# littlespray/StreamFlow

Measured on AMD Instinct MI355X. Metric: flow_fields_per_sec, higher is better.
Workload: dtype f16x2 / f16 mixed (activations fp16; weights fp16 in 24 of the 45 contraction / depthwise layers, hi+lo in the rest; fp32 accumulate); fp16 correlation volumes; 1 GPU; sintel_440x1024_T4_iters15; clips_per_launch=8, device_pinning=single device, flow_fields_per_clip=3, parallelism=replicas1, hip_graph=True, preset=config2_mixed, corr_volume=fp16 cells, single f16 MFMA product, fp32 accumulate, gma=flash (fused recompute, 1 MFMA product(s) per logit)

## Files before the change

### include/streamflow_hip.h

```cpp
#ifndef STREAMFLOW_HIP_H
#define STREAMFLOW_HIP_H

#include <stddef.h>
#include <stdint.h>

#ifdef __cplusplus
extern "C" {
#endif

#define SF_VERSION 122

enum {
    SF_OK = 0,
    SF_ERR_BAD_ARG = -1,
    SF_ERR_UNSUPPORTED = -2,
    SF_ERR_HIP = -3
};

int sf_version(void);
const char* sf_last_error(void);

int sf_coords_grid(float* out, int batch, int ht, int wd, void* stream);

int sf_bilinear_sampler(const float* img, const float* coords, float* out, float* mask_out,
                        int M, int C, int Hi, int Wi, int Ho, int Wo, void* stream);
// ... 119 lines not shown
                            int64_t out_img_stride, void* out_koct, int64_t out_koct_img_stride, int n_img, int P, void* stream);

typedef struct SfFfnPair {
    const void* X; int64_t strideX; int64_t ldx;
    const void* wstream; int64_t wstream_bytes;
    const float* bias1; const float* bias2; const float* dw_w; const float* dw_b;
    float* C; int64_t strideC; int64_t ldc;
    void* C16; int64_t strideC16; int64_t ldc16;
    int32_t N, batch, K1, H, M2, pm1, pm2, mode, gelu_out, c16_partial;
    float alpha1, alpha2;
    int32_t x_group; int64_t x_group_stride;
    const float* R32; int64_t strideR32, ldr32, r32_group_stride;
} SfFfnPair;
int sf_ffn_pair(const SfFfnPair* p, void* stream);
int sf_ffn_pair_frags(int K1, int M2, int pm1, int pm2);

typedef struct SfSkTail {
    const void* X; int64_t strideX; int64_t ldx;
    const void* wstream; int64_t wstream_bytes;
    const float* bias1; const float* bias2; const float* bias3;
    float* Y; int64_t strideY; int64_t ldy;
    void* Y16; int64_t strideY16; int64_t ldy16;
    int32_t N, batch, C, H, M2, pm, gelu_out, y16_partial;
    float alpha1, alpha2, alpha3;
} SfSkTail;
int sf_sk_tail(const SfSkTail* p, void* stream);
int sf_sk_tail_frags(int C, int H, int M2, int pm);
int sf_sk_tail_layout(int C, int H, int M2, int pm, int* stage, int* group, int* pw_one_unit);

typedef struct SfTemporalBlock {
// ... 82 lines not shown
```

### streamflow_amd/_lib.py

```python
from __future__ import annotations

import ctypes as C
import os
from typing import Optional

import torch

_HERE = os.path.dirname(os.path.abspath(__file__))
LIB_PATH = os.environ.get("SF_HIP_LIB") or os.path.join(_HERE, "libstreamflow_hip.so")

LAYOUT_K_MAJOR, LAYOUT_K_MINOR, LAYOUT_SPLIT_F16, LAYOUT_F16_K_MINOR, LAYOUT_F16_K_MAJOR, LAYOUT_F16_KOCT, LAYOUT_SPLIT_KOCT = 0, 1, 2, 3, 4, 5, 6
PRECISION_FP32, PRECISION_F16X3, PRECISION_F16X2, PRECISION_F16 = 0, 1, 2, 3
EPI_NONE, EPI_GELU, EPI_RELU, EPI_RES, EPI_RES_GELU, EPI_RES_GELU_DW1, EPI_AXPY = range(7)
ALGO_AUTO, ALGO_TILED, ALGO_BSTAT = 0, 1, 2

_vp, _i, _i64, _f = C.c_void_p, C.c_int, C.c_int64, C.c_float


class SfGemm(C.Structure):
    _fields_ = [
        ("A", _vp), ("B", _vp), ("C", _vp), ("bias", _vp), ("R", _vp), ("dw_w", _vp), ("dw_b", _vp), ("gamma", _vp),
        ("M", C.c_int32), ("N", C.c_int32), ("K", C.c_int32), ("batch", C.c_int32),
        ("lda", _i64), ("ldb", _i64), ("ldc", _i64), ("ldr", _i64),
        ("strideA", _i64), ("strideB", _i64), ("strideC", _i64), ("strideR", _i64),
# ... 97 lines not shown
    "sf_corr_build_blocked32_ws_bytes": (_i64, [_i, _i, _i, _i]),
    "sf_corr_build_blocked32": (_i, [_vp, _vp, _i64, _i64, _vp, _i64, _i, _i, _i, _i, _i, _vp, _i64, _vp]),
    "sf_corr_lookup_blocked32": (_i, [_vp, _i64, _vp, _vp, _i64, _i, _i, _i, _i, _vp]),
    "sf_gemm": (_i, [C.POINTER(SfGemm), _vp]),
    "sf_gemm_split_ws_floats": (_i64, [_i, _i, _i, _i]),
    "sf_gma_flash_ws_bytes": (_i64, [_i, _i]),
    "sf_gma_flash_pack_qk": (_i, [_vp, _i64, _vp, _i64, _i, _i, _f, _i, _vp]),
    "sf_gma_flash_aggregate": (_i, [_vp, _i64, _vp, _i64, _vp, _i64, _vp, _vp, _i64, _vp, _i64, _i, _i, _i, _i, _vp]),
    "sf_gma_flash_aggregate_f16v": (_i, [_vp, _i64, _vp, _i64, _vp, _i64, _vp, _vp, _i64, _vp, _i64, _i, _i, _i, _i, _vp]),
    "sf_gma_flash_project_v": (_i, [_vp, _i64, _vp, _i64, _i64, _vp, _vp, _i, _f, _i, _i, _i, _vp]),
    "sf_gma_stored_p_bytes": (_i64, [_i, _i]),
    "sf_gma_flash_store_p": (_i, [_vp, _i64, _vp, _i64, _i, _i, _i, _vp]),
    "sf_gma_stored_aggregate": (_i, [_vp, _i64, _vp, _i64, _vp, _i, _i64, _vp, _i64, _vp, _vp, _i64, _vp, _i64, _i, _i, _vp]),
    "sf_ffn_pair": (_i, [C.POINTER(SfFfnPair), _vp]),
    "sf_ffn_pair_frags": (_i, [_i, _i, _i, _i]),
    "sf_sk_tail": (_i, [C.POINTER(SfSkTail), _vp]),
    "sf_sk_tail_frags": (_i, [_i, _i, _i, _i]),
    "sf_sk_tail_layout": (_i, [_i, _i, _i, _i, C.POINTER(C.c_int), C.POINTER(C.c_int), C.POINTER(C.c_int)]),
    "sf_temporal_block": (_i, [C.POINTER(SfTemporalBlock), _vp]),
    "sf_temporal_block_frags": (_i, [_i]),
    "sf_mask_upsample": (_i, [C.POINTER(SfMaskUpsample), _vp]),
    "sf_mask_upsample_frags": (_i, [_i]),
    "sf_softmax_rows": (_i, [_vp, _i64, _i, _vp, _vp]),
    "sf_splitk_combine": (_i, [_vp, _i64, _i, _i64, _vp, _i64, _vp, _vp, _i64, _i, _i64, _vp]),
    "sf_dwconv_res_gelu": (_i, [_vp, _i64, _vp, _vp, _vp, _i64, _i, _i, _i, _i, _i, _i, _i, _vp]),
    "sf_dwconv_res_gelu_f16in": (_i, [_vp, _i64, _vp, _vp, _vp, _i64, _i, _i, _i, _i, _i, _i, _vp]),
    "sf_layernorm_cm": (_i, [_vp, _i64, _vp, _vp, _vp, _i64, _vp, _i64, _i, _i, _i, _f, _vp]),
    "sf_temporal_attn": (_i, [_vp, _vp, _vp, _i, _i, _i, _i, _vp]),
    "sf_temporal_attn_f16in": (_i, [_vp, _vp, _vp, _i, _i, _i, _i, _vp]),
    "sf_pack_koct": (_i, [_vp, _i64, _i, _i, _i, _vp, _i64, _vp]),
# ... 69 lines not shown
```

### streamflow_amd/build.py

```python
from __future__ import annotations

import os
import shutil
import subprocess
import sys
from concurrent.futures import ThreadPoolExecutor

HERE = os.path.dirname(os.path.abspath(__file__))
CSRC = os.path.join(HERE, "csrc")
OBJ = os.path.join(CSRC, "build")
LIB = os.path.join(HERE, "libstreamflow_hip.so")
ASAN_OBJ = os.path.join(CSRC, "build_asan")
ASAN_LIB = os.path.join(HERE, "libstreamflow_hip_asan.so")
SOURCES = ["misc.hip", "corr.hip", "corr_blocked.hip", "corr_blocked32.hip", "conv.hip", "gemm.hip", "gemm_split.hip", "gemm_bstat.hip", "ffn_pair.hip", "sk_tail.hip", "temporal.hip", "mask_upsample.hip", "attn.hip", "encoder.hip", "tile_blend.hip"]
HEADERS = [os.path.join(CSRC, "sf_common.h"), os.path.join(CSRC, "gemm_epilogue.h"), os.path.join(CSRC, "split_operand.h"),
           os.path.join(HERE, "..", "include", "streamflow_hip.h")]
FLAGS = ["--offload-arch=gfx950", "-O3", "-std=c++17", "-fPIC", "-fno-slp-vectorize", "-Wall",
         "-Wno-unused-function",
         "-Rpass-analysis=kernel-resource-usage"]
HOT_KERNELS = ("gemm_bstat", "ffn_pair_kernel", "sk_tail_kernel", "gma_flash_pipe_kernel", "gma_pv_kernel", "temporal_block_kernel", "mask_upsample_kernel", "gemm_bdirect_kernel", "gma_flash_kernel", "flash_project_v_kernel", "dwconv_mfma_kernel",
               "corr_lookup_blocked_kernel", "corr_build_blocked_kernel", "corr_lookup_blocked32_kernel", "corr_build_blocked32_kernel", "temporal_attn_kernel", "layernorm_cm_split_kernel",
               "flash_pack_v_kernel")


def hipcc() -> str:
    exe = shutil.which("hipcc") or "/opt/rocm/bin/hipcc"
    if not os.path.exists(exe):
        raise RuntimeError("hipcc not found; libstreamflow_hip.so cannot be built")
    return exe


def _stale(target: str, deps) -> bool:
    if not os.path.exists(target):
        return True
    t = os.path.getmtime(target)
# ... 169 lines not shown
```

### streamflow_amd/engine.py

```python
from __future__ import annotations

import contextlib
import os
from dataclasses import dataclass, fields, replace
from typing import Dict, List, Optional, Sequence, Tuple

import torch

from . import _lib, ops
from .ops import (EPI_AXPY, EPI_GELU, EPI_NONE, EPI_RELU, EPI_RES, EPI_RES_GELU, EPI_RES_GELU_DW1, LAYOUT_F16_K_MINOR,
                  LAYOUT_K_MAJOR, LAYOUT_K_MINOR, PackedLinear, Planes, Workspace)

HDIM = 128
COR_PLANES = 324


@dataclass(frozen=True)
class EngineOptions:
    parallel_branches: bool = True
    split_solo: int = 2
    split_uneven: bool = False
    auto_split_k: bool = True
    attn_chunk_rows: int = 0
    attn_k_splits: int = 3
    corr_blocked: bool = True
    corr_blocked32: bool = True
    shadows: bool = True
    shadow_fused: bool = True
    hidden_f16: bool = True
    hidden_koct: bool = True
    split_handover: bool = False
    pw_fold: bool = True
    koct_io: bool = True
    x2_f16: bool = True
    flash_stats: bool = True
    ffn_pairs: bool = True
    project_v: bool = True
    temporal_block: bool = True
    sk_tail: bool = True
    sk_tail_all: bool = False
    head_pairs: bool = False
    mask_upsample: bool = True
    clock_probe_us: int = 0
    setup_overlap: bool = True
    gma_per_chain: bool = True
    hybrid_store_pct: int = 50
    stored_auto_px: int = 16384
    stored_auto_max_gb: int = 16
    stored_p_max_gb: int = 64
    max_plans: int = 4

# ... 16 lines not shown

class SKBlockWeights:

    def __init__(self, sd: Dict[str, torch.Tensor], prefix: str, device):
        g = lambda n: sd[prefix + "." + n]
        self.ffn1_0 = PackedLinear(g("ffn1.0.weight"), g("ffn1.0.bias"), device)
        self.ffn1_2 = PackedLinear(g("ffn1.2.weight"), g("ffn1.2.bias"), device)
        self.pw = PackedLinear(g("pw.weight"), g("pw.bias"), device)
        wpw = g("pw.weight")
        eye = torch.eye(wpw.shape[0], dtype=wpw.dtype, device=wpw.device).reshape(wpw.shape[0], wpw.shape[0], *wpw.shape[2:])
        self.pw_res = PackedLinear(wpw + eye, g("pw.bias"), device)
        self.ffn2_0 = PackedLinear(g("ffn2.0.weight"), g("ffn2.0.bias"), device)
        self.ffn2_2 = PackedLinear(g("ffn2.2.weight"), g("ffn2.2.bias"), device)
        self.pair1 = ops.PackedPair(self.ffn1_0, self.ffn1_2)
        self.pair2 = ops.PackedPair(self.ffn2_0, self.ffn2_2)
        self.tail = ops.PackedTail(self.pw_res, self.ffn2_0, self.ffn2_2)
        self.c_in, self.c_mid, self.c_out = self.ffn1_0.K, self.ffn1_0.M, self.ffn2_2.M
        f32 = lambda t: t.detach().to(device=device, dtype=torch.float32).contiguous()
        w0 = g("conv_list.0.weight")
        if w0.shape[-1] != 1:
            raise RuntimeError("SKBlock: first depthwise kernel must be 1x1 (k_conv=[1,K]), got %s" % (tuple(w0.shape),))
        self.dw1_w = f32(w0.reshape(-1))
        self.dw1_b = f32(g("conv_list.0.bias"))
        wk = g("conv_list.1.weight")
        self.k = int(wk.shape[-1])
        self.dwk_w = f32(wk.reshape(wk.shape[0], -1))
        self.dwk_b = f32(g("conv_list.1.bias"))
        self.dw_single = False


# ... 17 lines not shown
    assert 0 <= i0 and i0 + cnt <= X.n_img
    step = X.img_stride // (2 if X.f16 else 1)
    assert not X.f16 or X.img_stride % 2 == 0
    sh = _sub(X.shadow, i0, cnt) if X.shadow is not None else None
    return replace(X, off=X.off + i0 * step, n_img=cnt, shadow=sh)


def _part(buf: Planes, i0: int, cnt: int) -> Planes:
    return replace(buf, off=buf.off + i0 * buf.img_stride, n_img=cnt)


def hidden_f16_ok(cx: ops.Ctx, P: int) -> bool:
    return cx.precision in (ops.PRECISION_F16X2, ops.PRECISION_F16) and P % 4 == 0 and cx.hidden_f16


def run_skblock(W: SKBlockWeights, X: Planes, Y: Planes, hid: Planes, xa: Planes, xb: Planes, h: int, w: int,
                final_gelu: bool = False, cx: Optional[ops.Ctx] = None) -> None:
    cx = ops._cx(cx)
    C = W.c_in
    assert X.rows == C and Y.rows == W.c_out and X.n_img == Y.n_img
    a, b = _scratch(xa, X.n_img, C), _scratch(xb, X.n_img, C)
    fold = hidden_f16_ok(cx, X.P) and cx.pw_fold
    if fold and cx.x2_f16:
        a = _scratch(xa, X.n_img, C, f16=True)
    head_pairs = cx.head_pairs and X.group and X.shadow is not None and X.n_img * X.P >= 4 * 7040
    if cx.ffn_pairs and a.f16 and ((X.f16 and X.koct) or head_pairs) and ops.ffn_pair_ok(W.pair1, X, 1, cx):
        ops.ffn_pair(W.pair1, X, a, 1, dw_w=W.dw1_w, dw_b=W.dw1_b, cx=cx)
    else:
        hidden = _handover(cx, hid, X.n_img, W.c_mid, X.P, consumer_rows=C)
        ops.gemm(W.ffn1_0, X, hidden, EPI_GELU, cx=cx)
        ops.gemm(W.ffn1_2, hidden, a, EPI_RES_GELU_DW1, R=X, dw_w=W.dw1_w, dw_b=W.dw1_b, cx=cx)
    if fold:
        b16 = _scratch(xb, X.n_img, C, f16=True)
        ops.dwconv_res_gelu(a, W.dwk_w, W.dwk_b, b16, h, w, W.k, single=W.dw_single, cx=cx)
        if (ops.sk_tail_ok(W.tail, b16, Y, cx) and W.c_in <= 256 and X.n_img * X.P >= 4 * 7040) or \
                (cx.sk_tail_all and ops.sk_tail_ok(W.tail, b16, Y, cx)):
            ops.sk_tail(W.tail, b16, Y, gelu_out=final_gelu, cx=cx)
            return
        a4 = _handover(cx, xa, X.n_img, C, X.P, consumer_rows=W.c_mid)
        ops.gemm(W.pw_res, b16, a4, EPI_GELU, cx=cx)
    else:
        ops.dwconv_res_gelu(a, W.dwk_w, W.dwk_b, b, h, w, W.k, single=W.dw_single, cx=cx)
        a4 = _handover(cx, xa, X.n_img, C, X.P, consumer_rows=W.c_mid, allow_koct=False)
        ops.gemm(W.pw, b, a4, EPI_RES_GELU, R=b, cx=cx)
    pair2_pays = W.c_in <= 128 or W.pair2.products(cx) == (1, 1) or (W.c_out <= 16 and head_pairs)
    if X.n_img * X.P < 4 * 7040 and not X.group:
        pair2_pays = True
    if (cx.ffn_pairs and pair2_pays and a4.f16 and a4.koct and ops.ffn_pair_ok(W.pair2, a4, 0, cx) and (not Y.f16 or Y.koct)):
        ops.ffn_pair(W.pair2, a4, Y, 0, gelu_out=final_gelu, cx=cx)
        return
    hidden = _handover(cx, hid, X.n_img, W.c_mid, X.P, consumer_rows=W.c_out)
    ops.gemm(W.ffn2_0, a4, hidden, EPI_GELU, cx=cx)
    ops.gemm(W.ffn2_2, hidden, Y, EPI_GELU if final_gelu else EPI_NONE, cx=cx)


class HotPathWeights:

    def __init__(self, sd: Dict[str, torch.Tensor], device, T: Optional[int] = None):
        sd = {(k[7:] if k.startswith("module.") else k): v for k, v in sd.items()}
# ... 196 lines not shown
        if self.gma_mode not in ("auto", "matrix", "flash", "stored", "hybrid"):
            raise RuntimeError(f"gma_mode must be auto, matrix, flash, stored or hybrid, got {self.gma_mode!r}")
        self.flash_qk_products = (int(flash_qk_products or 0)
                                  or {ops.PRECISION_F16X2: 2, ops.PRECISION_F16: 1}.get(self.precision, 3))
        if self.flash_qk_products not in (1, 2, 3):
            raise RuntimeError(f"flash_qk_products must be 1, 2 or 3, got {self.flash_qk_products}")
        self._side = torch.cuda.Stream(device=self.device)
        if int(self.options.clock_probe_us) > 0:
            self._probe_stream = torch.cuda.Stream(device=self.device)
            self.clock_counts = torch.zeros(2, dtype=torch.int64, device=self.device)
        self._chain_streams = [torch.cuda.Stream(device=self.device) for _ in range(3)]
        self.split_solo = int(self.options.split_solo)
        self.W = HotPathWeights(state_dict, self.device, T)
        self.single_layers = tuple(single_layers or ())
        self.W.set_single("all" if self.single_layers == ("all",) else self.single_layers)
        if (self.options.ffn_pairs or self.options.sk_tail) and self.precision in (ops.PRECISION_F16X2, ops.PRECISION_F16):
            cxp = ops.Ctx(precision=self.precision)
            with torch.cuda.device(self.device):
                for b in HotPathWeights.SK_BLOCKS:
                    blk = getattr(self.W, b)
                    for pair in (blk.pair1, blk.pair2) if self.options.ffn_pairs else ():
                        if (pair.K1, pair.M2) in ops.PAIR_SHAPES[0] | ops.PAIR_SHAPES[1]:
                            pair.stream(*pair.products(cxp))
                    if self.options.sk_tail and blk.tail.built(blk.tail.products(cxp)):
                        blk.tail.stream(blk.tail.products(cxp))
                torch.cuda.synchronize(self.device)
        if self.options.mask_upsample and self.precision in (ops.PRECISION_F16X2, ops.PRECISION_F16) and self.W.mask_pack.built():
            with torch.cuda.device(self.device):
                self.W.mask_pack.stream(self.W.mask_pack.products(ops.Ctx(precision=self.precision)))
                torch.cuda.synchronize(self.device)
        if self.options.temporal_block and self.precision in (ops.PRECISION_F16X2, ops.PRECISION_F16) and self.W.temporal.built():
            pm = self.W.temporal.products(ops.Ctx(precision=self.precision))
            if pm is not None:
                with torch.cuda.device(self.device):
                    self.W.temporal.stream(pm)
                    torch.cuda.synchronize(self.device)
        self.use_graph = use_graph
        self._plans: Dict[Tuple[int, int, int, int], _Plan] = {}
# ... 21 lines not shown
                       corr_blocked=self.corr_blocked, corr_blocked32=self.corr_blocked32,
                       koct_io=self.options.koct_io and self.options.hidden_koct,
                       stored_p=((self.gma_mode in ("stored", "hybrid") or auto_stored) and self.options.flash_stats),
                       stored_frac=(1.0 if (self.gma_mode == "stored" or auto_stored) else float(self.options.hybrid_store_pct) / 100.0),
                       stored_p_max_bytes=int(self.options.stored_p_max_gb) << 30)
            pl.auto_stored = bool(auto_stored and pl.pbuf is not None)
        self._plans[key] = pl
        return pl

    def _ctx(self, pl: _Plan) -> ops.Ctx:
        o = self.options
        return ops.Ctx(precision=self.precision,
                       split_ws=pl.splitws.tensor().view(-1) if self.auto_split_k else None,
                       shadows=o.shadows, shadow_fused=o.shadow_fused, flash_stats=o.flash_stats,
                       hidden_f16=o.hidden_f16, hidden_koct=o.hidden_koct, split_handover=o.split_handover, pw_fold=o.pw_fold, x2_f16=o.x2_f16,
                       ffn_pairs=o.ffn_pairs, head_pairs=o.head_pairs, sk_tail=o.sk_tail, sk_tail_all=o.sk_tail_all)

    @staticmethod
    def _flash_ws_sub(pl: _Plan, i0: int, cnt: int) -> torch.Tensor:
        if i0 == 0 and cnt == pl.n:
            return pl.flash_ws
        ib = ops.gma_flash_img_bytes(pl.P)
        return pl.flash_ws[i0 * ib:(i0 + cnt) * ib]

    def _attention_rows(self, cx: ops.Ctx, pl: _Plan, i0: int, rows: int) -> None:
        P, n = pl.P, pl.n
        ops.gemm_raw(cx, A=pl.qk.ptr + 4 * i0, B=pl.qk.ptr + 4 * HDIM * P, C=pl.attn.data_ptr(), M=rows, N=P, K=HDIM,
                     batch=n, lda=P, ldb=P, ldc=P, strideA=pl.qk.img_stride, strideB=pl.qk.img_stride,
                     strideC=pl.attn_rows * P, a_layout=LAYOUT_K_MAJOR, b_layout=LAYOUT_K_MAJOR,
                     alpha=float(HDIM) ** -0.5, epilogue=EPI_NONE)
        if rows == pl.attn_rows:
# ... 303 lines not shown
```

### streamflow_amd/ops.py

```python
from __future__ import annotations

import ctypes as C
import math
import os
from dataclasses import dataclass, replace
from typing import Optional, Sequence

import torch

from . import _lib
from ._lib import (EPI_AXPY, EPI_GELU, EPI_NONE, EPI_RELU, EPI_RES, EPI_RES_GELU, EPI_RES_GELU_DW1,
                   LAYOUT_K_MAJOR, LAYOUT_K_MINOR, LAYOUT_SPLIT_F16, LAYOUT_F16_K_MINOR, PRECISION_F16, PRECISION_F16X2, PRECISION_F16X3,
                   PRECISION_FP32,
                   SfGemm)

PRECISION = PRECISION_F16X3
_PRECISION_NAMES = {"fp32": PRECISION_FP32, "f16x3": PRECISION_F16X3, "f16x2": PRECISION_F16X2, "f16": PRECISION_F16}


def set_precision(mode) -> int:
    global PRECISION
    prev = PRECISION
    PRECISION = _PRECISION_NAMES[mode] if isinstance(mode, str) else int(mode)
    if PRECISION not in (PRECISION_FP32, PRECISION_F16X3, PRECISION_F16X2, PRECISION_F16):
# ... 8 lines not shown

@dataclass(frozen=True)
class Ctx:
    precision: int
    split_ws: Optional[torch.Tensor] = None
    shadows: bool = True
    shadow_fused: bool = True
    flash_stats: bool = True
    hidden_f16: bool = True
    hidden_koct: bool = True
    split_handover: bool = False
    pw_fold: bool = True
    x2_f16: bool = True
    ffn_pairs: bool = True
    head_pairs: bool = False
    sk_tail: bool = True
    sk_tail_all: bool = False

    def no_split(self) -> "Ctx":
        return self if self.split_ws is None else replace(self, split_ws=None)


def _cx(cx: Optional["Ctx"]) -> "Ctx":
    return cx if cx is not None else Ctx(PRECISION)


class Profiler:

    def __init__(self):
        self.records = []
# ... 229 lines not shown
        h1, l1 = self._split(self.first, hp * 32, nk1 * 32)
        h2, l2 = self._split(self.second, nt2 * 16, hp * 32)
        dev = h1.device
        planes1 = [l1, h1] if pm1 == 2 else [h1]
        f1 = torch.stack([w.view(hp, 2, 16, nk1, 4, 8) for w in planes1], dim=0)
        f1 = f1.permute(1, 2, 4, 0, 5, 3, 6).reshape(hp, 2 * nk1 * pm1, 64 * 8)
        kq = torch.arange(4, device=dev).view(4, 1)
        i = torch.arange(8, device=dev).view(1, 8)
        perm = torch.where(i < 4, 4 * kq + i, 16 + 4 * kq + i - 4).reshape(-1)
        planes2 = [l2, h2] if pm2 == 2 else [h2]
        f2 = torch.stack([w.view(nt2, 16, hp, 32)[..., perm].reshape(nt2, 16, hp, 4, 8) for w in planes2], dim=0)
        f2 = f2.permute(3, 1, 0, 4, 2, 5).reshape(hp, nt2 * pm2, 64 * 8)
        pad = torch.zeros(hp, fpad - f1.shape[1] - f2.shape[1], 64 * 8, dtype=torch.float16, device=dev)
        st = torch.cat([f1, f2, pad], dim=1).contiguous().view(-1)
        assert st.numel() * 2 == hp * fpad * 1024
        self._streams[key] = st
        return st


class PackedTail:

    S = 16

    def __init__(self, pw_res: "PackedLinear", f0: "PackedLinear", f2: "PackedLinear"):
        assert pw_res.M == pw_res.K == f0.K and f0.M == f2.K and not (pw_res.conv3x3 or f0.conv3x3 or f2.conv3x3)
        self.layers = (pw_res, f0, f2)
        self.C, self.H, self.M2 = pw_res.K, f0.M, f2.M
        self._streams = {}

    def products(self, cx: "Ctx") -> Optional[int]:
# ... 293 lines not shown
        g.C16, g.strideC16, g.ldc16 = Y.ptr, Y.img_stride, Y.P
    else:
        g.C, g.strideC, g.ldc = Y.ptr, Y.img_stride, Y.P
        out_bytes = 4.0
        if Y.shadow is not None and cx.shadows:
            sh = Y.shadow
            g.C16, g.strideC16, g.ldc16 = sh.ptr, sh.img_stride, sh.P
            g.c16_partial = 1 if pair.M2 % 8 else 0
            out_bytes = 6.0
    n, P = X.n_img, X.P
    flops = 2.0 * n * P * (pair.K1 * pair.H + pair.H * pair.M2)
    mf = 2.0 * n * P * (pair.K1 * pair.H * pm1 + pair.H * pair.M2 * pm2)
    nbytes = n * P * (2.0 * pair.K1 * (2 if mode == 1 else 1) + out_bytes * pair.M2) + 2.0 * (pair.K1 * pair.H * pm1 + pair.H * pair.M2 * pm2)
    name = "ffn_pair" if not PROFILE_SHAPES else f"ffn_pair K{pair.K1} H{pair.H} M{pair.M2} b{n} m{mode}"
    _launch(name, flops, nbytes, lambda: _lib.check(_lib.load().sf_ffn_pair(C.byref(g), _lib.stream()), "sf_ffn_pair"),
            products=mf / flops)
    if g.C and not g.C16:
        refresh_shadow(Y, cx)


def new_shadow(X: Planes, device) -> Planes:
    assert not X.f16 and X.group == 0
    noct = (X.rows + 7) // 8
    base = torch.zeros(X.n_img * noct * X.P * 4, dtype=torch.float32, device=device)
    return Planes(base, 0, noct * X.P * 8, X.n_img, X.rows, X.P, f16=True, koct=True)


@on_tensor_device
def pack_koct(X: Planes, Y: Planes) -> None:
    assert Y.f16 and Y.koct and not X.f16 and X.group == 0 and (X.rows, X.P, X.n_img) == (Y.rows, Y.P, Y.n_img)
# ... 577 lines not shown
```

Baseline: 387.1 flow-fields/s.

## Add fused FFN chain kernel keeping hidden tile in registers across both GEMMs

Adds a new ffn_chain kernel that computes the two pointwise layers of an FFN block in one pass. Each hidden 32-row tile is produced by MFMA, passed through GELU, converted to f16 fragments and consumed straight away by the second GEMM. Weights stream through a three-stage LDS ring using buffer-load-to-LDS, and a mode-1 epilogue applies the residual, depthwise and GELU steps. This is meant to replace the existing ffn_pair path for suitable shapes and cut hidden-activation traffic, at the cost of high register pressure and more complex weight packing.

```diff
diff --git a/include/streamflow_hip.h b/include/streamflow_hip.h
--- a/include/streamflow_hip.h
+++ b/include/streamflow_hip.h
@@ -8,7 +8,7 @@
 extern "C" {
 #endif
 
-#define SF_VERSION 122
+#define SF_VERSION 123
 
 enum {
     SF_OK = 0,
@@ -158,6 +158,8 @@
 } SfFfnPair;
 int sf_ffn_pair(const SfFfnPair* p, void* stream);
 int sf_ffn_pair_frags(int K1, int M2, int pm1, int pm2);
+int sf_ffn_chain(const SfFfnPair* p, void* stream);
+int sf_ffn_chain_frags(int K1, int H, int M2, int pm1, int pm2);
 
 typedef struct SfSkTail {
     const void* X; int64_t strideX; int64_t ldx;
diff --git a/streamflow_amd/_lib.py b/streamflow_amd/_lib.py
--- a/streamflow_amd/_lib.py
+++ b/streamflow_amd/_lib.py
@@ -135,6 +135,8 @@
     "sf_gma_stored_aggregate": (_i, [_vp, _i64, _vp, _i64, _vp, _i, _i64, _vp, _i64, _vp, _vp, _i64, _vp, _i64, _i, _i, _vp]),
     "sf_ffn_pair": (_i, [C.POINTER(SfFfnPair), _vp]),
     "sf_ffn_pair_frags": (_i, [_i, _i, _i, _i]),
+    "sf_ffn_chain": (_i, [C.POINTER(SfFfnPair), _vp]),
+    "sf_ffn_chain_frags": (_i, [_i, _i, _i, _i, _i]),
     "sf_sk_tail": (_i, [C.POINTER(SfSkTail), _vp]),
     "sf_sk_tail_frags": (_i, [_i, _i, _i, _i]),
     "sf_sk_tail_layout": (_i, [_i, _i, _i, _i, C.POINTER(C.c_int), C.POINTER(C.c_int), C.POINTER(C.c_int)]),
diff --git a/streamflow_amd/build.py b/streamflow_amd/build.py
--- a/streamflow_amd/build.py
+++ b/streamflow_amd/build.py
@@ -12,13 +12,13 @@
 LIB = os.path.join(HERE, "libstreamflow_hip.so")
 ASAN_OBJ = os.path.join(CSRC, "build_asan")
 ASAN_LIB = os.path.join(HERE, "libstreamflow_hip_asan.so")
-SOURCES = ["misc.hip", "corr.hip", "corr_blocked.hip", "corr_blocked32.hip", "conv.hip", "gemm.hip", "gemm_split.hip", "gemm_bstat.hip", "ffn_pair.hip", "sk_tail.hip", "temporal.hip", "mask_upsample.hip", "attn.hip", "encoder.hip", "tile_blend.hip"]
+SOURCES = ["misc.hip", "corr.hip", "corr_blocked.hip", "corr_blocked32.hip", "conv.hip", "gemm.hip", "gemm_split.hip", "gemm_bstat.hip", "ffn_pair.hip", "ffn_chain.hip", "sk_tail.hip", "temporal.hip", "mask_upsample.hip", "attn.hip", "encoder.hip", "tile_blend.hip"]
 HEADERS = [os.path.join(CSRC, "sf_common.h"), os.path.join(CSRC, "gemm_epilogue.h"), os.path.join(CSRC, "split_operand.h"),
            os.path.join(HERE, "..", "include", "streamflow_hip.h")]
 FLAGS = ["--offload-arch=gfx950", "-O3", "-std=c++17", "-fPIC", "-fno-slp-vectorize", "-Wall",
          "-Wno-unused-function",
          "-Rpass-analysis=kernel-resource-usage"]
-HOT_KERNELS = ("gemm_bstat", "ffn_pair_kernel", "sk_tail_kernel", "gma_flash_pipe_kernel", "gma_pv_kernel", "temporal_block_kernel", "mask_upsample_kernel", "gemm_bdirect_kernel", "gma_flash_kernel", "flash_project_v_kernel", "dwconv_mfma_kernel",
+HOT_KERNELS = ("gemm_bstat", "ffn_pair_kernel", "ffn_chain_kernel", "sk_tail_kernel", "gma_flash_pipe_kernel", "gma_pv_kernel", "temporal_block_kernel", "mask_upsample_kernel", "gemm_bdirect_kernel", "gma_flash_kernel", "flash_project_v_kernel", "dwconv_mfma_kernel",
                "corr_lookup_blocked_kernel", "corr_build_blocked_kernel", "corr_lookup_blocked32_kernel", "corr_build_blocked32_kernel", "temporal_attn_kernel", "layernorm_cm_split_kernel",
                "flash_pack_v_kernel")
 
diff --git a/streamflow_amd/csrc/ffn_chain.hip b/streamflow_amd/csrc/ffn_chain.hip
--- /dev/null
+++ b/streamflow_amd/csrc/ffn_chain.hip
@@ -0,0 +1,383 @@
+#include "sf_common.h"
+#include <type_traits>
+
+namespace {
+
+typedef _Float16 f16x8 __attribute__((ext_vector_type(8)));
+typedef _Float16 f16x4 __attribute__((ext_vector_type(4)));
+typedef float f32x16 __attribute__((ext_vector_type(16)));
+typedef float f32x4 __attribute__((ext_vector_type(4)));
+typedef unsigned int u32x2 __attribute__((ext_vector_type(2)));
+typedef __attribute__((address_space(3))) void* lds_ptr;
+using sf::f32x2;
+
+constexpr int kThreads = 256, kWaves = 4;
+constexpr int BN = 128;
+constexpr int S = 16;
+constexpr int kStage = S * 1024;
+constexpr int RING = 3;
+constexpr int PCS = S / kWaves;
+constexpr int kOob = 1 << 30;
+constexpr int kMaxH = 960, kMaxM = 384;
+
+struct ChainArgs {
+    SfFfnPair p;
+    int ntile;
+    int nh;
+    int x_span;
+    int64_t w_bytes;
+};
+
+template <int N>
+__device__ __forceinline__ void wait_vm() { __builtin_amdgcn_s_waitcnt((N & 15) | 0x0F70 | ((N >> 4) << 14)); }
+
+template <int I, int N, class F>
+__device__ __forceinline__ void static_for(F&& f) {
+    if constexpr (I < N) {
+        f(std::integral_constant<int, I>{});
+        static_for<I + 1, N>(f);
+    }
+}
+
+template <int NP>
+__device__ __forceinline__ void gelu_poly_n(f32x2 (&x)[NP]) {
+    f32x2 xc[NP], t[NP], p[NP];
+#pragma unroll
+    for (int i = 0; i < NP; ++i) {
+        xc[i][0] = __builtin_amdgcn_fmed3f(x[i][0], -4.2426405f, 4.2426405f);
+        xc[i][1] = __builtin_amdgcn_fmed3f(x[i][1], -4.2426405f, 4.2426405f);
+        t[i] = xc[i] * xc[i];
+        p[i] = sf::splat2(1.12535e-10f);
+    }
+    constexpr float c[8] = {-1.074371e-08f, 4.5365834e-07f, -1.12924145e-05f, 0.0001871811f, -0.0022188f, 0.019636236f,
+                            -0.13269384f, 0.79780626f};
+#pragma unroll
+    for (int k = 0; k < 8; ++k)
+#pragma unroll
+        for (int i = 0; i < NP; ++i) p[i] = __builtin_elementwise_fma(p[i], t[i], sf::splat2(c[k]));
+#pragma unroll
+    for (int i = 0; i < NP; ++i) {
+        const f32x2 h = sf::splat2(0.5f) * __builtin_elementwise_max(x[i], sf::splat2(-4.2426405f));
+        x[i] = __builtin_elementwise_fma(h, xc[i] * p[i], h);
+    }
+}
+
+template <int NP>
+__device__ __forceinline__ void tile_to_frags(const f32x16& acc, float alpha, f16x8& f0, f16x8& f1) {
+#pragma unroll
+    for (int s = 0; s < 2; ++s) {
+        f16x8 h;
+#pragma unroll
+        for (int c = 0; c < 4; c += NP) {
+            f32x2 v[NP];
+#pragma unroll
+            for (int q = 0; q < NP; ++q) {
+                v[q][0] = alpha * acc[8 * s + 2 * (c + q)];
+                v[q][1] = alpha * acc[8 * s + 2 * (c + q) + 1];
+            }
+            gelu_poly_n<NP>(v);
+#pragma unroll
+            for (int q = 0; q < NP; ++q) {
+                h[2 * (c + q)] = (_Float16)v[q][0];
+                h[2 * (c + q) + 1] = (_Float16)v[q][1];
+            }
+        }
+        if (s == 0) f0 = h; else f1 = h;
+    }
+}
+
+constexpr int chain_regs(int NK1, int NM, int MODE) { return (MODE == 1 ? 2 * NM : NK1) * 4 + NM * 16; }
+
+template <int NK1, int NM, int PM1, int PM2, int MODE>
+__global__ __launch_bounds__(kThreads, chain_regs(NK1, NM, MODE) <= 212 ? 2 : 1) void ffn_chain_kernel(const ChainArgs a) {
+    const SfFfnPair& g = a.p;
+    constexpr int NX = MODE == 1 ? 2 * NM : NK1;
+    static_assert(NX >= NK1, "mode 1 needs M2 == K1");
+    constexpr int NA = NK1 * PM1, NB = 2 * NM * PM2, TF = NA + NB;
+    constexpr int U = (TF + S - 1) / S;
+    constexpr int GNP = chain_regs(NK1, NM, MODE) > 160 ? 2 : 4;
+    __shared__ __attribute__((aligned(1024))) char smem[RING * kStage + (kMaxH + kMaxM) * 4];
+    float* sb1 = reinterpret_cast<float*>(smem + RING * kStage);
+    float* sb2 = sb1 + kMaxH;
+    float* sdw = reinterpret_cast<float*>(smem);
+    float* sdb = sdw + kMaxM;
+    const int tid = threadIdx.x, lane = tid & 63;
+    const int wave = __builtin_amdgcn_readfirstlane(tid >> 6);
+    const int khalf = lane >> 5, l31 = lane & 31;
+    const int tile = blockIdx.x % a.ntile, z = blockIdx.x / a.ntile;
+    const int n = tile * BN + wave * 32 + l31, nc = min(n, g.N - 1);
+
+    const __amdgpu_buffer_rsrc_t rw = __builtin_amdgcn_make_buffer_rsrc(const_cast<void*>(g.wstream), 0, (int)a.w_bytes, 0x00020000);
+    const int last_stage = (int)(a.w_bytes / kStage) - 1;
+    auto issue_stage = [&](int s, int slot) {
+        const int sc = min(s, last_stage);
+#pragma unroll
+        for (int i = 0; i < PCS; ++i) {
+            const int piece = wave + kWaves * i;
+            __builtin_amdgcn_raw_ptr_buffer_load_lds(rw, (lds_ptr)(smem + slot * kStage + piece * 1024), 16, lane * 16,
+                                                     sc * kStage + piece * 1024, 0, 0);
+        }
+    };
+#pragma unroll
+    for (int i = 0; i < RING - 1; ++i) issue_stage(i, i);
+
+    for (int i = tid; i < a.nh * 32; i += kThreads) sb1[i] = (i < g.H && g.bias1) ? g.bias1[i] : 0.f;
+    for (int i = tid; i < NM * 32; i += kThreads) sb2[i] = (i < g.M2 && g.bias2) ? g.bias2[i] : 0.f;
+
+    const int noct = (g.K1 + 7) / 8;
+    const __amdgpu_buffer_rsrc_t rx = __builtin_amdgcn_make_buffer_rsrc(
+        const_cast<char*>(reinterpret_cast<const char*>(g.X)) + (int64_t)z * g.strideX * 2, 0, a.x_span, 0x00020000);
+    f16x8 x[NX];
+#pragma unroll
+    for (int s = 0; s < NX; ++s) {
+        const int oc = 2 * s + khalf;
+        x[s] = __builtin_bit_cast(f16x8, __builtin_amdgcn_raw_buffer_load_b128(rx, oc < noct ? (khalf * (int)g.ldx + nc) * 16 : kOob,
+                                                                              2 * s * (int)g.ldx * 16, 0));
+    }
+    wait_vm<0>();
+    __syncthreads();
+
+    int gs = 0, slot = 0;
+    auto run_unit = [&](auto&& body) {
+        static_for<0, U>([&](auto st_tag) {
+            constexpr int st = decltype(st_tag)::value;
+            issue_stage(gs + RING - 1, slot == 0 ? RING - 1 : slot - 1);
+            const char* sp = smem + slot * kStage + lane * 16;
+            static_for<0, S>([&](auto i_tag) {
+                constexpr int i = decltype(i_tag)::value;
+                body(std::integral_constant<int, st * S + i>{}, sp + i * 1024);
+            });
+            {
+                constexpr int nm = (TF - st * S) < 0 ? 0 : ((TF - st * S) > S ? S : (TF - st * S));
+                constexpr int kAhead = 3;
+                __builtin_amdgcn_sched_group_barrier(0x002, 2, 0);
+                __builtin_amdgcn_sched_group_barrier(0x100, nm < kAhead ? nm : kAhead, 0);
+#pragma unroll
+                for (int i = 0; i < nm; ++i) {
+                    if (st * S + i == NA) __builtin_amdgcn_sched_group_barrier(0x002, 200, 0);
+                    __builtin_amdgcn_sched_group_barrier(0x008, 1, 0);
+                    if (i + kAhead < nm) __builtin_amdgcn_sched_group_barrier(0x100, 1, 0);
+                }
+            }
+            asm volatile("s_waitcnt lgkmcnt(0)" ::: "memory");
+            wait_vm<PCS * (RING - 2)>();
+            __builtin_amdgcn_s_barrier();
+            asm volatile("" ::: "memory");
+            __builtin_amdgcn_sched_barrier(0);
+            ++gs;
+            slot = (slot == RING - 1) ? 0 : slot + 1;
+        });
+    };
+    auto bias_rows = [&](const float* sb, int t32) {
+        f32x16 acc;
+#pragma unroll
+        for (int j = 0; j < 4; ++j) {
+            const f32x4 b4 = *reinterpret_cast<const f32x4*>(sb + t32 * 32 + 8 * j + 4 * khalf);
+#pragma unroll
+            for (int e = 0; e < 4; ++e) acc[4 * j + e] = b4[e];
+        }
+        return acc;
+    };
+    auto bias_chan = [&](const float* sb, int t32) {
+        f32x16 acc;
+#pragma unroll
+        for (int h = 0; h < 4; ++h) {
+            const f32x4 b4 = *reinterpret_cast<const f32x4*>(sb + t32 * 32 + 16 * (h >> 1) + 8 * khalf + 4 * (h & 1));
+#pragma unroll
+            for (int e = 0; e < 4; ++e) acc[4 * h + e] = b4[e];
+        }
+        return acc;
+    };
+
+    f32x16 acc2[NM];
+#pragma unroll
+    for (int m = 0; m < NM; ++m) acc2[m] = MODE == 1 ? bias_chan(sb2, m) : bias_rows(sb2, m);
+    for (int th = 0; th < a.nh; ++th) {
+        f32x16 acch = bias_rows(sb1, th);
+        f16x8 hf[2] = {};
+        run_unit([&](auto f_tag, const char* p) {
+            constexpr int f = decltype(f_tag)::value;
+            if constexpr (f < TF) {
+                if constexpr (f == NA) tile_to_frags<GNP>(acch, g.alpha1, hf[0], hf[1]);
+                if constexpr (f < NA) {
+                    acch = __builtin_amdgcn_mfma_f32_32x32x16_f16(*reinterpret_cast<const f16x8*>(p), x[f / PM1], acch, 0, 0, 0);
+                } else {
+                    constexpr int q = (f - NA) / PM2, s_ = q / NM, m = q % NM;
+                    acc2[m] = __builtin_amdgcn_mfma_f32_32x32x16_f16(*reinterpret_cast<const f16x8*>(p), hf[s_], acc2[m], 0, 0, 0);
+                }
+            }
+        });
+    }
+    wait_vm<0>();
+
+    if constexpr (MODE == 0) {
+        const __amdgpu_buffer_rsrc_t rc32 = __builtin_amdgcn_make_buffer_rsrc(
+            g.C ? reinterpret_cast<char*>(g.C) + (int64_t)z * g.strideC * 4 : nullptr, 0,
+            g.C ? (int)(((int64_t)(g.M2 - 1) * g.ldc + g.N) * 4) : 0, 0x00020000);
+        const __amdgpu_buffer_rsrc_t rc16 = __builtin_amdgcn_make_buffer_rsrc(
+            g.C16 ? reinterpret_cast<char*>(g.C16) + (int64_t)z * g.strideC16 * 2 : nullptr, 0,
+            g.C16 ? (int)((int64_t)((g.M2 + 7) / 8) * g.ldc16 * 16) : 0, 0x00020000);
+        const int lane_c32 = (n < g.N) ? (4 * khalf * (int)g.ldc + n) * 4 : kOob;
+        const int lane_k16 = (n < g.N) ? n * 16 + khalf * 8 : kOob;
+        const int k4 = 4 * khalf;
+        auto rows_left = [&](int r) { return __builtin_amdgcn_readfirstlane(g.M2 - r); };
+        auto rows_left8 = [&](int r) { return __builtin_amdgcn_readfirstlane((g.M2 + 7) / 8 * 8 - r); };
+#pragma unroll
+        for (int m = 0; m < NM; ++m)
+#pragma unroll
+            for (int j0 = 0; j0 < 4; j0 += 2) {
+                f32x2 v[4];
+#pragma unroll
+                for (int q = 0; q < 4; ++q) {
+                    const int j = j0 + (q >> 1), e = (q & 1) * 2;
+                    v[q][0] = g.alpha2 * acc2[m][4 * j + e];
+                    v[q][1] = g.alpha2 * acc2[m][4 * j + e + 1];
+                }
+                if (g.gelu_out) {
+                    if (g.C) {
+#pragma unroll
+                        for (int q = 0; q < 4; ++q) v[q] = sf::gelu_erf2(v[q]);
+                    } else {
+                        gelu_poly_n<4>(v);
+                    }
+                }
+#pragma unroll
+                for (int jj = 0; jj < 2; ++jj) {
+                    const int j = j0 + jj, rb = m * 32 + 8 * j;
+                    const float o[4] = {v[2 * jj][0], v[2 * jj][1], v[2 * jj + 1][0], v[2 * jj + 1][1]};
+                    if (g.C) {
+#pragma unroll
+                        for (int e = 0; e < 4; ++e)
+                            __builtin_amdgcn_raw_buffer_store_b32(__builtin_bit_cast(unsigned, o[e]), rc32,
+                                                                  (k4 < rows_left(rb + e)) ? lane_c32 : kOob, (rb + e) * (int)g.ldc * 4, 0);
+                    }
+                    if (g.C16) {
+                        f16x4 h;
+#pragma unroll
+                        for (int e = 0; e < 4; ++e) h[e] = (_Float16)o[e];
+                        const int so = (rb >> 3) * (int)g.ldc16 * 16;
+                        const bool full = g.c16_partial ? (k4 < rows_left(rb + 3)) : (k4 < rows_left8(rb));
+                        __builtin_amdgcn_raw_buffer_store_b64(__builtin_bit_cast(u32x2, h), rc16, full ? lane_k16 : kOob, so, 0);
+                        if (g.c16_partial && (g.M2 & 3) && rb + 8 > g.M2 && rb < g.M2) {
+#pragma unroll
+                            for (int e = 0; e < 3; ++e) {
+                                const _Float16 he = h[e];
+                                const bool part = k4 < rows_left(rb) && !(k4 < rows_left(rb + 3)) && k4 < rows_left(rb + e);
+                                __builtin_amdgcn_raw_buffer_store_b16(__builtin_bit_cast(unsigned short, he), rc16,
+                                                                      part ? lane_k16 + e * 2 : kOob, so, 0);
+                            }
+                        }
+                    }
+                }
+            }
+    } else {
+        __syncthreads();
+        for (int i = tid; i < NM * 32; i += kThreads) {
+            sdw[i] = (i < g.M2) ? g.dw_w[i] : 0.f;
+            sdb[i] = (i < g.M2) ? g.dw_b[i] : 0.f;
+        }
+        __syncthreads();
+        const __amdgpu_buffer_rsrc_t rc = __builtin_amdgcn_make_buffer_rsrc(
+            reinterpret_cast<char*>(g.C16) + (int64_t)z * g.strideC16 * 2, 0, (int)(((int64_t)(g.M2 - 1) * g.ldc16 + g.N) * 2), 0x00020000);
+        const int vrow = (n < g.N) ? (8 * khalf * (int)g.ldc16 + n) * 2 : kOob;
+#pragma unroll
+        for (int t = 0; t < NM; ++t)
+#pragma unroll
+            for (int hh = 0; hh < 2; ++hh) {
+                const int c0 = 32 * t + 16 * hh + 8 * khalf;
+                const f32x4 w0 = *reinterpret_cast<const f32x4*>(sdw + c0), w1 = *reinterpret_cast<const f32x4*>(sdw + c0 + 4);
+                const f32x4 b0 = *reinterpret_cast<const f32x4*>(sdb + c0), b1 = *reinterpret_cast<const f32x4*>(sdb + c0 + 4);
+                const f16x8 xr = x[2 * t + hh];
+#pragma unroll
+                for (int q = 0; q < 4; ++q) {
+                    const int r = 8 * hh + 2 * q;
+                    f32x2 v, res, w2, b2;
+                    v[0] = g.alpha2 * acc2[t][r]; v[1] = g.alpha2 * acc2[t][r + 1];
+                    res[0] = (float)xr[2 * q]; res[1] = (float)xr[2 * q + 1];
+                    w2[0] = q < 2 ? w0[2 * q] : w1[2 * q - 4]; w2[1] = q < 2 ? w0[2 * q + 1] : w1[2 * q - 3];
+                    b2[0] = q < 2 ? b0[2 * q] : b1[2 * q - 4]; b2[1] = q < 2 ? b0[2 * q + 1] : b1[2 * q - 3];
+                    const f32x2 x1 = sf::gelu_poly2(res + v);
+                    const f32x2 x2 = sf::gelu_poly2(x1 + (w2 * x1 + b2));
+#pragma unroll
+                    for (int e = 0; e < 2; ++e) {
+                        const _Float16 he = (_Float16)x2[e];
+                        const int ch = c0 + 2 * q + e;
+                        __builtin_amdgcn_raw_buffer_store_b16(__builtin_bit_cast(unsigned short, he), rc, ch < g.M2 ? vrow : kOob,
+                                                              (32 * t + 16 * hh + 2 * q + e) * (int)g.ldc16 * 2, 0);
+                    }
+                }
+            }
+    }
+}
+
+struct Shape { int K1, M2, mode, NK1, NM; };
+constexpr Shape kShapes[] = {{128, 128, 1, 8, 4}, {256, 256, 1, 16, 8}, {324, 324, 1, 21, 11}, {324, 256, 0, 21, 8}, {640, 128, 0, 40, 4}};
+
+inline const Shape* find_shape(int K1, int M2) {
+    for (const Shape& s : kShapes)
+        if (s.K1 == K1 && s.M2 == M2) return &s;
+    return nullptr;
+}
+
+inline bool built(const Shape* s, int pm1, int pm2) {
+    if (!s) return false;
+    if (s->mode == 1) return (pm1 == 1 && pm2 == 1) || (pm1 == 2 && pm2 == 2);
+    if (s->K1 == 324) return pm1 == 2 && (pm2 == 1 || pm2 == 2);
+    return pm1 == 2 && pm2 == 2;
+}
+
+}
+
+extern "C" int sf_ffn_chain_frags(int K1, int H, int M2, int pm1, int pm2) {
+    const Shape* s = find_shape(K1, M2);
+    if (!built(s, pm1, pm2) || H <= 0 || H > kMaxH) return 0;
+    const int tf = s->NK1 * pm1 + 2 * s->NM * pm2;
+    return (H + 31) / 32 * ((tf + S - 1) / S * S);
+}
+
+extern "C" int sf_ffn_chain(const SfFfnPair* p, void* stream) {
+    SF_REQUIRE(p && p->X && p->wstream, "sf_ffn_chain: null pointer");
+    const SfFfnPair& g = *p;
+    SF_REQUIRE(g.K1 > 0 && g.H > 0 && g.M2 > 0 && g.N > 0 && g.batch > 0, "sf_ffn_chain: bad dims");
+    SF_REQUIRE(g.x_group == 0 && !g.R32, "sf_ffn_chain: grouped views and fp32 residuals are sf_ffn_pair's");
+    const Shape* s = find_shape(g.K1, g.M2);
+    const int frags = sf_ffn_chain_frags(g.K1, g.H, g.M2, g.pm1, g.pm2);
+    SF_REQUIRE(frags > 0 && s->mode == g.mode, "sf_ffn_chain: shape K1=%d H=%d M2=%d mode %d products (%d, %d) not built", g.K1, g.H,
+               g.M2, g.mode, g.pm1, g.pm2);
+    SF_REQUIRE((reinterpret_cast<uintptr_t>(g.X) & 15) == 0 && (g.strideX & 7) == 0 && g.ldx >= g.N &&
+                   (reinterpret_cast<uintptr_t>(g.wstream) & 15) == 0,
+               "sf_ffn_chain: X (k-octet planes) and the weight stream must be 16-byte aligned, strideX %% 8 == 0, ldx >= N");
+    const int64_t lim = (int64_t)1 << 30;
+    const int64_t x_span = (int64_t)((g.K1 + 7) / 8) * g.ldx * 16;
+    SF_REQUIRE(x_span < lim, "sf_ffn_chain: input image larger than 1 GiB");
+    if (g.mode == 0) {
+        SF_REQUIRE(g.C || g.C16, "sf_ffn_chain: mode 0 needs C (fp32 planes) and / or C16 (k-octet planes)");
+        SF_REQUIRE(!g.C16 || ((reinterpret_cast<uintptr_t>(g.C16) & 15) == 0 && (g.strideC16 & 7) == 0 && g.ldc16 >= g.N &&
+                              (int64_t)((g.M2 + 7) / 8) * g.ldc16 * 16 < lim),
+                   "sf_ffn_chain: C16 (k-octet planes) must be 16-byte aligned, strideC16 %% 8 == 0, ldc16 >= N, image < 1 GiB");
+        SF_REQUIRE(!g.C || (g.ldc >= g.N && ((int64_t)(g.M2 - 1) * g.ldc + g.N) * 4 < lim), "sf_ffn_chain: C: ldc >= N, image < 1 GiB");
+    } else {
+        SF_REQUIRE(g.C16 && g.dw_w && g.dw_b, "sf_ffn_chain: mode 1 needs C16 (fp16 rows), dw_w and dw_b");
+        SF_REQUIRE(g.ldc16 >= g.N && ((int64_t)(g.M2 - 1) * g.ldc16 + g.N) * 2 < lim, "sf_ffn_chain: C16 rows: ldc16 >= N, image < 1 GiB");
+    }
+    ChainArgs a;
+    a.p = g;
+    a.ntile = sf::ceil_div(g.N, BN);
+    a.nh = (g.H + 31) / 32;
+    a.x_span = (int)x_span;
+    a.w_bytes = (int64_t)frags * 1024;
+    SF_REQUIRE(g.wstream_bytes >= a.w_bytes && a.w_bytes < lim, "sf_ffn_chain: weight stream too small (need %lld bytes) or > 1 GiB",
+               (long long)a.w_bytes);
+    SF_REQUIRE((int64_t)a.ntile * g.batch < ((int64_t)1 << 31), "sf_ffn_chain: grid too large");
+    const dim3 grid((unsigned)((int64_t)a.ntile * g.batch)), block(kThreads);
+    hipStream_t st = (hipStream_t)stream;
+    const int pm = g.pm1 * 10 + g.pm2;
+#define SF_CHAIN(NK1_, NM_, PM1_, PM2_, MODE_) hipLaunchKernelGGL((ffn_chain_kernel<NK1_, NM_, PM1_, PM2_, MODE_>), grid, block, 0, st, a)
+    if (s->K1 == 128) { if (pm == 11) SF_CHAIN(8, 4, 1, 1, 1); else SF_CHAIN(8, 4, 2, 2, 1); }
+    else if (s->K1 == 256) { if (pm == 11) SF_CHAIN(16, 8, 1, 1, 1); else SF_CHAIN(16, 8, 2, 2, 1); }
+    else if (s->mode == 1) { if (pm == 11) SF_CHAIN(21, 11, 1, 1, 1); else SF_CHAIN(21, 11, 2, 2, 1); }
+    else if (s->K1 == 324) { if (pm == 21) SF_CHAIN(21, 8, 2, 1, 0); else SF_CHAIN(21, 8, 2, 2, 0); }
+    else SF_CHAIN(40, 4, 2, 2, 0);
+#undef SF_CHAIN
+    return sf::check_launch("sf_ffn_chain");
+}
diff --git a/streamflow_amd/engine.py b/streamflow_amd/engine.py
--- a/streamflow_amd/engine.py
+++ b/streamflow_amd/engine.py
@@ -35,6 +35,7 @@
     x2_f16: bool = True
     flash_stats: bool = True
     ffn_pairs: bool = True
+    ffn_chain: bool = True
     project_v: bool = True
     temporal_block: bool = True
     sk_tail: bool = True
@@ -81,6 +82,8 @@
         self.ffn2_2 = PackedLinear(g("ffn2.2.weight"), g("ffn2.2.bias"), device)
         self.pair1 = ops.PackedPair(self.ffn1_0, self.ffn1_2)
         self.pair2 = ops.PackedPair(self.ffn2_0, self.ffn2_2)
+        self.chain1 = ops.PackedChain(self.ffn1_0, self.ffn1_2)
+        self.chain2 = ops.PackedChain(self.ffn2_0, self.ffn2_2)
         self.tail = ops.PackedTail(self.pw_res, self.ffn2_0, self.ffn2_2)
         self.c_in, self.c_mid, self.c_out = self.ffn1_0.K, self.ffn1_0.M, self.ffn2_2.M
         f32 = lambda t: t.detach().to(device=device, dtype=torch.float32).contiguous()
@@ -128,6 +131,13 @@
     return cx.precision in (ops.PRECISION_F16X2, ops.PRECISION_F16) and P % 4 == 0 and cx.hidden_f16
 
 
+CHAIN_SHAPES = set()
+
+
+def chain_pays(chain: "ops.PackedChain") -> bool:
+    return (chain.K1, chain.M2) in CHAIN_SHAPES
+
+
 def run_skblock(W: SKBlockWeights, X: Planes, Y: Planes, hid: Planes, xa: Planes, xb: Planes, h: int, w: int,
                 final_gelu: bool = False, cx: Optional[ops.Ctx] = None) -> None:
     cx = ops._cx(cx)
@@ -138,7 +148,10 @@
     if fold and cx.x2_f16:
         a = _scratch(xa, X.n_img, C, f16=True)
     head_pairs = cx.head_pairs and X.group and X.shadow is not None and X.n_img * X.P >= 4 * 7040
-    if cx.ffn_pairs and a.f16 and ((X.f16 and X.koct) or head_pairs) and ops.ffn_pair_ok(W.pair1, X, 1, cx):
+    big = X.n_img * X.P >= 4 * 7040
+    if big and a.f16 and chain_pays(W.chain1) and ops.ffn_chain_ok(W.chain1, X, 1, cx):
+        ops.ffn_chain(W.chain1, X, a, 1, dw_w=W.dw1_w, dw_b=W.dw1_b, cx=cx)
+    elif cx.ffn_pairs and a.f16 and ((X.f16 and X.koct) or head_pairs) and ops.ffn_pair_ok(W.pair1, X, 1, cx):
         ops.ffn_pair(W.pair1, X, a, 1, dw_w=W.dw1_w, dw_b=W.dw1_b, cx=cx)
     else:
         hidden = _handover(cx, hid, X.n_img, W.c_mid, X.P, consumer_rows=C)
@@ -157,6 +170,9 @@
         ops.dwconv_res_gelu(a, W.dwk_w, W.dwk_b, b, h, w, W.k, single=W.dw_single, cx=cx)
         a4 = _handover(cx, xa, X.n_img, C, X.P, consumer_rows=W.c_mid, allow_koct=False)
         ops.gemm(W.pw, b, a4, EPI_RES_GELU, R=b, cx=cx)
+    if big and a4.f16 and a4.koct and chain_pays(W.chain2) and ops.ffn_chain_ok(W.chain2, a4, 0, cx) and (not Y.f16 or Y.koct):
+        ops.ffn_chain(W.chain2, a4, Y, 0, gelu_out=final_gelu, cx=cx)
+        return
     pair2_pays = W.c_in <= 128 or W.pair2.products(cx) == (1, 1) or (W.c_out <= 16 and head_pairs)
     if X.n_img * X.P < 4 * 7040 and not X.group:
         pair2_pays = True
@@ -383,7 +399,7 @@
         self.W = HotPathWeights(state_dict, self.device, T)
         self.single_layers = tuple(single_layers or ())
         self.W.set_single("all" if self.single_layers == ("all",) else self.single_layers)
-        if (self.options.ffn_pairs or self.options.sk_tail) and self.precision in (ops.PRECISION_F16X2, ops.PRECISION_F16):
+        if (self.options.ffn_pairs or self.options.sk_tail or self.options.ffn_chain) and self.precision in (ops.PRECISION_F16X2, ops.PRECISION_F16):
             cxp = ops.Ctx(precision=self.precision)
             with torch.cuda.device(self.device):
                 for b in HotPathWeights.SK_BLOCKS:
@@ -391,6 +407,9 @@
                     for pair in (blk.pair1, blk.pair2) if self.options.ffn_pairs else ():
                         if (pair.K1, pair.M2) in ops.PAIR_SHAPES[0] | ops.PAIR_SHAPES[1]:
                             pair.stream(*pair.products(cxp))
+                    for chain in (blk.chain1, blk.chain2) if self.options.ffn_chain else ():
+                        if chain_pays(chain) and chain.frags(*chain.products(cxp)) > 0:
+                            chain.stream(*chain.products(cxp))
                     if self.options.sk_tail and blk.tail.built(blk.tail.products(cxp)):
                         blk.tail.stream(blk.tail.products(cxp))
                 torch.cuda.synchronize(self.device)
@@ -442,7 +461,7 @@
                        split_ws=pl.splitws.tensor().view(-1) if self.auto_split_k else None,
                        shadows=o.shadows, shadow_fused=o.shadow_fused, flash_stats=o.flash_stats,
                        hidden_f16=o.hidden_f16, hidden_koct=o.hidden_koct, split_handover=o.split_handover, pw_fold=o.pw_fold, x2_f16=o.x2_f16,
-                       ffn_pairs=o.ffn_pairs, head_pairs=o.head_pairs, sk_tail=o.sk_tail, sk_tail_all=o.sk_tail_all)
+                       ffn_pairs=o.ffn_pairs, ffn_chain=o.ffn_chain, head_pairs=o.head_pairs, sk_tail=o.sk_tail, sk_tail_all=o.sk_tail_all)
 
     @staticmethod
     def _flash_ws_sub(pl: _Plan, i0: int, cnt: int) -> torch.Tensor:
diff --git a/streamflow_amd/ops.py b/streamflow_amd/ops.py
--- a/streamflow_amd/ops.py
+++ b/streamflow_amd/ops.py
@@ -46,6 +46,7 @@
     x2_f16: bool = True
     ffn_pairs: bool = True
     head_pairs: bool = False
+    ffn_chain: bool = True
     sk_tail: bool = True
     sk_tail_all: bool = False
 
@@ -305,6 +306,50 @@
         pad = torch.zeros(hp, fpad - f1.shape[1] - f2.shape[1], 64 * 8, dtype=torch.float16, device=dev)
         st = torch.cat([f1, f2, pad], dim=1).contiguous().view(-1)
         assert st.numel() * 2 == hp * fpad * 1024
+        self._streams[key] = st
+        return st
+
+
+class PackedChain(PackedPair):
+
+    def __init__(self, first: "PackedLinear", second: "PackedLinear"):
+        super().__init__(first, second)
+        self.mode = 1 if self.M2 == self.K1 else 0
+
+    def frags(self, pm1: int, pm2: int) -> int:
+        return int(_lib.load().sf_ffn_chain_frags(self.K1, self.H, self.M2, pm1, pm2))
+
+    def stream(self, pm1: int, pm2: int) -> torch.Tensor:
+        key = (pm1, pm2)
+        if key in self._streams:
+            return self._streams[key]
+        if torch.cuda.is_available() and torch.cuda.is_current_stream_capturing():
+            raise RuntimeError("PackedChain.stream: weight stream requested for the first time inside a graph capture; build it "
+                               "before (HotPathEngine does at construction)")
+        total = self.frags(pm1, pm2)
+        if total <= 0:
+            raise RuntimeError(f"PackedChain: K1={self.K1} H={self.H} M2={self.M2} products {key} not built (sf_ffn_chain_frags)")
+        nk1, nm, nh = (self.K1 + 15) // 16, (self.M2 + 31) // 32, (self.H + 31) // 32
+        h1, l1 = self._split(self.first, nh * 32, nk1 * 16)
+        h2, l2 = self._split(self.second, nm * 32, nh * 32)
+        dev = h1.device
+        if self.mode == 1:
+            p = torch.arange(nm * 32, device=dev)
+            perm = (p & ~12) | ((p >> 1) & 4) | ((p << 1) & 8)
+            h2, l2 = h2[perm], l2[perm]
+        planes1 = [l1, h1] if pm1 == 2 else [h1]
+        f1 = torch.stack([w.view(nh, 32, nk1, 2, 8) for w in planes1], dim=0)
+        f1 = f1.permute(1, 3, 0, 4, 2, 5).reshape(nh, nk1 * pm1, 512)
+        khalf = torch.arange(2, device=dev).view(2, 1)
+        i = torch.arange(8, device=dev).view(1, 8)
+        acc_order = torch.cat([16 * s_ + ((i & 3) + 8 * (i >> 2) + 4 * khalf).reshape(-1) for s_ in (0, 1)])
+        planes2 = [l2, h2] if pm2 == 2 else [h2]
+        f2 = torch.stack([w.view(nm * 32, nh, 32)[:, :, acc_order].reshape(nm, 32, nh, 2, 2, 8) for w in planes2], dim=0)
+        f2 = f2.permute(3, 4, 1, 0, 5, 2, 6).reshape(nh, 2 * nm * pm2, 512)
+        per = total // nh
+        pad = torch.zeros(nh, per - f1.shape[1] - f2.shape[1], 512, dtype=torch.float16, device=dev)
+        st = torch.cat([f1, f2, pad], dim=1).contiguous().view(-1)
+        assert st.numel() == total * 512
         self._streams[key] = st
         return st
 
@@ -628,6 +673,62 @@
     nbytes = n * P * (2.0 * pair.K1 * (2 if mode == 1 else 1) + out_bytes * pair.M2) + 2.0 * (pair.K1 * pair.H * pm1 + pair.H * pair.M2 * pm2)
     name = "ffn_pair" if not PROFILE_SHAPES else f"ffn_pair K{pair.K1} H{pair.H} M{pair.M2} b{n} m{mode}"
     _launch(name, flops, nbytes, lambda: _lib.check(_lib.load().sf_ffn_pair(C.byref(g), _lib.stream()), "sf_ffn_pair"),
+            products=mf / flops)
+    if g.C and not g.C16:
+        refresh_shadow(Y, cx)
+
+
+def ffn_chain_ok(chain: Optional[PackedChain], X: Planes, mode: int, cx: Optional["Ctx"] = None) -> bool:
+    cx = _cx(cx)
+    if chain is None or not cx.ffn_chain or chain.mode != mode or cx.precision not in (PRECISION_F16X2, PRECISION_F16) or \
+            not (cx.shadows and cx.hidden_f16 and cx.hidden_koct):
+        return False
+    src = X if (X.f16 and X.koct) else (None if mode == 1 else X.shadow)
+    if src is None or src.group or X.group or X.P % 4:
+        return False
+    return chain.frags(*chain.products(cx)) > 0
+
+
+@on_tensor_device
+def ffn_chain(chain: PackedChain, X: Planes, Y: Planes, mode: int, dw_w: Optional[torch.Tensor] = None,
+              dw_b: Optional[torch.Tensor] = None, gelu_out: bool = False, cx: Optional["Ctx"] = None) -> None:
+    cx = _cx(cx)
+    assert ffn_chain_ok(chain, X, mode, cx)
+    src = X if (X.f16 and X.koct) else X.shadow
+    pm1, pm2 = chain.products(cx)
+    st = chain.stream(pm1, pm2)
+    g = _lib.SfFfnPair()
+    g.X, g.strideX, g.ldx = src.ptr, src.img_stride, src.P
+    g.wstream, g.wstream_bytes = st.data_ptr(), st.numel() * 2
+    A1, A2 = chain.first, chain.second
+    g.bias1 = None if A1.bias_split is None else A1.bias_split.data_ptr()
+    g.bias2 = None if A2.bias_split is None else A2.bias_split.data_ptr()
+    g.alpha1, g.alpha2 = 1.0 / A1.split_scale, 1.0 / A2.split_scale
+    g.N, g.batch, g.K1, g.H, g.M2 = X.P, X.n_img, chain.K1, chain.H, chain.M2
+    g.pm1, g.pm2, g.mode, g.gelu_out = pm1, pm2, int(mode), int(bool(gelu_out))
+    assert Y.n_img == X.n_img and Y.P == X.P and Y.rows == chain.M2 and Y.group == 0
+    out_bytes = 2.0
+    if mode == 1:
+        assert Y.f16 and not Y.koct and dw_w is not None and dw_b is not None
+        g.dw_w, g.dw_b = dw_w.data_ptr(), dw_b.data_ptr()
+        g.C16, g.strideC16, g.ldc16 = Y.ptr, Y.img_stride, Y.P
+    elif Y.f16:
+        assert Y.koct
+        g.C16, g.strideC16, g.ldc16 = Y.ptr, Y.img_stride, Y.P
+    else:
+        g.C, g.strideC, g.ldc = Y.ptr, Y.img_stride, Y.P
+        out_bytes = 4.0
+        if Y.shadow is not None and cx.shadows:
+            sh = Y.shadow
+            g.C16, g.strideC16, g.ldc16 = sh.ptr, sh.img_stride, sh.P
+            g.c16_partial = 1 if chain.M2 % 8 else 0
+            out_bytes = 6.0
+    n, P = X.n_img, X.P
+    flops = 2.0 * n * P * (chain.K1 * chain.H + chain.H * chain.M2)
+    mf = 2.0 * n * P * (chain.K1 * chain.H * pm1 + chain.H * chain.M2 * pm2)
+    nbytes = n * P * (2.0 * chain.K1 + out_bytes * chain.M2) + 2.0 * (chain.K1 * chain.H * pm1 + chain.H * chain.M2 * pm2)
+    name = "ffn_chain" if not PROFILE_SHAPES else f"ffn_chain K{chain.K1} H{chain.H} M{chain.M2} b{n} m{mode}"
+    _launch(name, flops, nbytes, lambda: _lib.check(_lib.load().sf_ffn_chain(C.byref(g), _lib.stream()), "sf_ffn_chain"),
             products=mf / flops)
     if g.C and not g.C16:
         refresh_shadow(Y, cx)
```

Measured after the change: 387.2 flow-fields/s (median of 6 runs). About the same (+0.0%).
